# ELEKTRONN/ELEKTRONN2

Measured on AMD Instinct MI355X. Metric: training_input_voxels_per_sec, higher is better.
Workload: dtype f32; 1 GPU; neuro3d_lite (1,1,23,183,183)->(1,2,10,37,37) fwd+bwd+Adam, 1 sample/GPU; parallelism=dp1, hipgraph=True, steps_per_launch=10

## Files before the change

elektronn2_amd/backend.py:

```python
from __future__ import annotations

import ctypes as C
import os
from typing import Optional, Sequence

import numpy as np
import torch

_HERE = os.path.dirname(os.path.abspath(__file__))
LIB_PATH = os.environ.get("E2HIP_LIB") or os.path.join(_HERE, "libe2hip.so")

ACT = {"lin": 0, "linear": 0, "relu": 1, "tanh": 2, "sigmoid": 3, "sig": 3, "logistic": 3,
       "abs": 4, "elu": 5, "selu": 6, "soft+": 7}


class E2Error(RuntimeError):
    pass


POOL_MODE = {'avg': 1, 'sum': 2}


class Tensor5(C.Structure):
    _fields_ = [("ptr", C.c_void_p),
# ... 69 lines not shown
        "e2_conv3d_wgrad_acc": (C.c_int, [vp, P5, P5, fp, i, i, i]),
        "e2_conv3d_wgrad_pad": (C.c_int, [vp, P5, P5, fp, i, i, i, i]),
        "e2_pack_job_bytes": (sz, []),
        "e2_pack_job_fill": (C.c_int, [vp, fp, vp, i, i, i, i, i, i]),
        "e2_pack_job_set_rows": (C.c_int, [vp, i]),
        "e2_pack_job_set_stride": (C.c_int, [vp, i]),
        "e2_set_image_rows": (C.c_int, [vp, i]),
        "e2_conv3d_pack_multi": (C.c_int, [vp, vp, i]),
        "e2_conv3d_pack_multi_ex": (C.c_int, [vp, vp, i, i]),
        "e2_head_supported": (C.c_int, [i, i]),
        "e2_head_fwd": (C.c_int, [vp, P5, fp, fp, i, P5, P5, fp]),
        "e2_head_bwd_workspace_bytes": (C.c_size_t, [i, i, i, i, i, i]),
        "e2_tail_supported": (C.c_int, [i, i, i]),
        "e2_tail_workspace_bytes": (C.c_size_t, [i, i, i, i, i, i, i]),
        "e2_tail_fwd_bwd": (C.c_int, [vp, P5, fp, fp, fp, i, fp, fp, i, P5, P5, P5, P5, i, P5, fp, fp,
                                      C.c_void_p, C.c_size_t, C.POINTER(C.c_int)]),
        "e2_tail_reduce": (C.c_int, [vp, C.c_void_p, i, i, i, fp, fp, fp, fp, fp, i, fp]),
        "e2_head_bwd": (C.c_int, [vp, P5, fp, P5, P5, fp, P5, i, fp, fp, fp, C.c_void_p,
                                  C.c_size_t]),
        "e2_malis_loss_weights": (C.c_int, [i, C.c_void_p, i, C.c_void_p, C.c_void_p,
                                            C.c_void_p, i, C.c_void_p]),
        "e2_malis_connected_components": (C.c_int, [i, i, C.c_void_p, C.c_void_p, C.c_void_p,
                                                    i, C.c_void_p]),
        "e2_warp_slice": (C.c_int, [vp, P5, C.POINTER(C.c_float), i, C.c_uint,
                                    C.POINTER(C.c_int), C.POINTER(C.c_float), P5]),
        "e2_grey_augment": (C.c_int, [vp, fp, C.c_size_t, C.c_float, C.c_float, C.c_float]),
        "e2_stream_fork": (C.c_int, [vp, C.c_void_p]),
        "e2_stream_join": (C.c_int, [vp, C.c_void_p]),
        "e2_conv1_supported": (C.c_int, [i, i, i, i, i, i, i]),
        "e2_conv1_pool_act_fwd": (C.c_int, [vp, P5, fp, fp, i, i, i, i, i, i, P5]),
        "e2_conv1_bwd_workspace_bytes": (C.c_size_t, [i, i, i, i, i, i, i]),
        "e2_conv1_pool_act_bwd": (C.c_int, [vp, P5, fp, fp, P5, i, i, i, i, i, fp, fp,
                                            C.c_void_p, C.c_size_t]),
        "e2_pool_bias_act_fwd": (C.c_int, [vp, P5, fp, i, i, i, i, P5]),
        "e2_conv3d_fwd_packed_parts": (C.c_int, [vp, P5, vp, i, i, i, i, P5, C.c_int64, i,
                                                 C.POINTER(C.c_int)]),
        "e2_conv3d_dgrad_packed_parts": (C.c_int, [vp, P5, vp, i, i, i, i, P5, C.c_int64, i,
                                                   C.POINTER(C.c_int)]),
        "e2_pool_bias_act_fwd_parts": (C.c_int, [vp, P5, C.c_int64, i, fp, i, i, i, i, P5]),
        "e2_pool_bias_act_bwd_parts": (C.c_int, [vp, P5, C.c_int64, i, P5, fp, i, i, i, i, P5, fp]),
        "e2_bias_act_bwd_out_parts": (C.c_int, [vp, P5, C.c_int64, i, P5, i, P5, fp]),
        "e2_pool_bias_act_bwd": (C.c_int, [vp, P5, P5, fp, i, i, i, i, P5, fp]),
        "e2_maxpool3d_fwd": (C.c_int, [vp, P5, i, i, i, P5]),
        "e2_maxpool3d_bwd": (C.c_int, [vp, P5, P5, i, i, i, P5, i]),
        "e2_pool3d_lin_fwd": (C.c_int, [vp, P5, i, i, i, i, i, i, i, P5]),
        "e2_pool3d_lin_bwd": (C.c_int, [vp, P5, i, i, i, i, i, i, i, P5, i]),
        "e2_upconv3d_workspace_bytes": (sz, [i, i, i, i, i, i, i, i, i]),
        "e2_upconv3d_fwd": (C.c_int, [vp, P5, fp, fp, i, i, i, i, i, P5, vp, sz]),
        "e2_upconv3d_bwd": (C.c_int, [vp, P5, fp, P5, P5, i, i, i, i, P5, fp, fp, vp, sz]),
        "e2_upconv3d_image_bytes": (sz, [i, i, i, i, i]),
        "e2_upconv3d_fwd_packed": (C.c_int, [vp, P5, fp, fp, i, i, i, i, i, P5]),
        "e2_upconv3d_bwd_packed": (C.c_int, [vp, P5, fp, P5, P5, i, i, i, i, P5, fp, fp, vp, sz, i]),
        "e2_transpose_ncdhw_to_ndhwc": (C.c_int, [vp, P5, fp]),
        "e2_transpose_ndhwc_to_ncdhw": (C.c_int, [vp, fp, P5]),
        "e2_copy5": (C.c_int, [vp, P5, P5, i]),
        "e2_set_dgrad_zinset": (C.c_int, [vp, i]),
        "e2_pad5": (C.c_int, [vp, P5, P5, i, i, i, C.c_float, i]),
        "e2_fill": (C.c_int, [vp, fp, sz, C.c_float]),
        "e2_softmax_nll_fwd": (C.c_int, [vp, P5, P5, P5, fp]),
        "e2_softmax_nll_bwd": (C.c_int, [vp, P5, P5, fp, P5, fp]),
        "e2_softmax_nll_fwd_w": (C.c_int, [vp, P5, P5, P5, fp, PW]),
        "e2_softmax_nll_bwd_w": (C.c_int, [vp, P5, P5, fp, P5, fp, PW]),
        "e2_softmax_nll_grouped_fwd": (C.c_int, [vp, P5, P5, P5, i, fp]),
        "e2_softmax_nll_grouped_bwd": (C.c_int, [vp, P5, P5, i, fp, P5, fp]),
        "e2_head_fwd_w": (C.c_int, [vp, P5, fp, fp, i, P5, P5, fp, PW]),
        "e2_head_bwd_w": (C.c_int, [vp, P5, fp, P5, P5, fp, P5, i, fp, fp, fp, C.c_void_p,
# ... 380 lines not shown
                                          int(getattr(jobs_dev, 'max_taps', 248))),
             "e2_conv3d_pack_multi_ex")

    @staticmethod
    def conv1_supported(cin, k, pool):
        return bool(_lib.e2_conv1_supported(cin, k[0], k[1], k[2], pool[0], pool[1], pool[2]))

    def conv1_pool_act_fwd(self, x, w, bias, pool, act, out):
        _chk(_lib.e2_conv1_pool_act_fwd(self.h, C.byref(t5(x)), _fp(w), _fp(bias), w.shape[0],
                                        w.shape[3], w.shape[4], pool[1], pool[2], ACT[act],
                                        C.byref(t5(out))), "e2_conv1_pool_act_fwd")

    def conv1_pool_act_fwd_bf16(self, x, w, bias, pool, act, out, next_xb, next_kg):
        _chk(_lib.e2_conv1_pool_act_fwd_bf16(self.h, C.byref(t5(x)), _fp(w), _fp(bias), w.shape[0],
                                             w.shape[3], w.shape[4], pool[1], pool[2], ACT[act],
                                             C.byref(t5(out)), C.c_void_p(next_xb.data_ptr()),
                                             int(next_kg)), "e2_conv1_pool_act_fwd_bf16")

    @staticmethod
    def conv1_bwd_ws_bytes(dout_shape, k):
        n, cout, d, ho, wo = (int(v) for v in dout_shape)
        return int(_lib.e2_conv1_bwd_workspace_bytes(n, cout, d, ho, wo, k[1], k[2]))

    def conv1_pool_act_bwd(self, x, w, bias, dout, pool, act, dw, dbias, ws=None):
        if ws is None:
            ws = torch.empty(self.conv1_bwd_ws_bytes(dout.shape, w.shape[2:]) // 4 + 16,
                             dtype=torch.float32, device=self.device)
        _chk(_lib.e2_conv1_pool_act_bwd(self.h, C.byref(t5(x)), _fp(w), _fp(bias),
                                        C.byref(t5(dout)), w.shape[3], w.shape[4], pool[1],
                                        pool[2], ACT[act], _fp(dw), _fp(dbias),
                                        C.c_void_p(ws.data_ptr()), ws.numel() * 4),
             "e2_conv1_pool_act_bwd")

    def pool_bias_act_fwd(self, y, bias, pool, act, out):
        _chk(_lib.e2_pool_bias_act_fwd(self.h, C.byref(t5(y)), _fp(bias), pool[0], pool[1],
                                       pool[2], ACT[act], C.byref(t5(out))),
             "e2_pool_bias_act_fwd")

    def pool_bias_act_bwd(self, dout, y, bias, pool, act, dy, dbias):
        _chk(_lib.e2_pool_bias_act_bwd(self.h, C.byref(t5(dout)), C.byref(t5(y)), _fp(bias),
                                       pool[0], pool[1], pool[2], ACT[act], C.byref(t5(dy)),
                                       _fp(dbias)), "e2_pool_bias_act_bwd")

    def act_fwd(self, pre, bias, act, out):
        _chk(_lib.e2_act_fwd(self.h, C.byref(t5(pre)), _fp(bias), ACT[act], C.byref(t5(out))),
             "e2_act_fwd")

    def loss_partials(self, pred):
        n = int(_lib.e2_loss_partials(self.h, C.byref(t5(pred))))
        if n <= 0:
            raise E2Error("e2_loss_partials: empty prediction %s" % (tuple(pred.shape),))
        return n

    def loss_fwd(self, term, pred, sig, target, partials):
        if partials.numel() < 4 * self.loss_partials(pred):
            raise E2Error("loss_fwd: the partials slab is too small for this prediction")
        _chk(_lib.e2_loss_fwd(self.h, C.byref(term), C.byref(t5(pred)),
                              None if sig is None else C.byref(t5(sig)), C.byref(t5(target)),
                              _fp(partials)), "e2_loss_fwd")

    def loss_mix(self, terms, partials, n_tot, mix, coef, term_loss, count, loss_out):
        k = len(terms)
        if not (len(partials) == len(n_tot) == k):
            raise E2Error("loss_mix: %d terms, %d slabs, %d sizes" % (k, len(partials), len(n_tot)))
        if k > MAX_LOSS_TERMS:
            raise E2Error("loss_mix: %d terms, at most %d are supported" % (k, MAX_LOSS_TERMS))
# ... 473 lines not shown
```

elektronn2_amd/csrc/conv_first.hip:

```cpp
#include "common.hpp"
#include <algorithm>

struct First {
  const float* x;
  const float* w;
  const float* bias;
  float* out;
  const float* dout;
  float* dw;
  float* dbias;
  int N, Cout, D, Ho, Wo;
  long xsN, xsD, xsH;
  long osN, osC, osD, osH;
  int act;
  int tilesX, tilesY;
};

template <int KH, int KW, int PY, int PX>
__device__ __forceinline__ float first_conv(const float (&win)[PY + KH - 1][PX + KW - 1],
                                            const float* __restrict__ wc, int a, int b) {
  float s = 0.f;
#pragma unroll
  for (int ty = 0; ty < KH; ++ty)
#pragma unroll
// ... 220 lines not shown

static int conv1_fwd(e2_ctx* ctx, const e2_tensor5* x, const float* w, const float* bias, int cout,
                     int kh, int kw, int py, int px, int act, const e2_tensor5* out, void* next_xb,
                     int next_kg) {
  E2_REQUIRE(ctx && w && bias, "conv1_pool_act_fwd: null argument");
  const int v = first_supported(1, kh, kw, 1, py, px);
  E2_REQUIRE(v, "conv1_pool_act_fwd: unsupported kernel/pool %dx%d / %dx%d", kh, kw, py, px);
  First p{};
  if (int rc = first_fill(p, x, out, cout, kh, kw, py, px, "conv1_pool_act_fwd")) return rc;
  p.w = w; p.bias = bias; p.out = out->ptr; p.act = act;
  if (e2i_firstm_mg(cout) && (next_xb || !e2_dbg_env("E2_FIRST_VALU")))
    return e2i_firstm_fwd(ctx, v, x, w, bias, cout, py, px, act, out, next_xb, next_kg);
  E2_REQUIRE(!next_xb, "conv1_pool_act_fwd_bf16: %d output channels (matrix-core form: <= 32)", cout);
  const long nTiles = (long)p.N * p.D * p.tilesY * p.tilesX;
  const int grid = (int)std::min<long>(nTiles, ctx->num_cu * 8);
  if (v == 1)
    hipLaunchKernelGGL((first_fwd_kernel<4, 4, 2, 2>), dim3(grid), dim3(256), 0, ctx->stream, p, (int)nTiles);
  else if (v == 2)
    hipLaunchKernelGGL((first_fwd_kernel<6, 6, 2, 2>), dim3(grid), dim3(256), 0, ctx->stream, p, (int)nTiles);
  else
    hipLaunchKernelGGL((first_fwd_kernel<3, 3, 1, 1>), dim3(grid), dim3(256), 0, ctx->stream, p, (int)nTiles);
  E2_CHECK_HIP(hipGetLastError());
  return 0;
}

extern "C" size_t e2_conv1_bwd_workspace_bytes(int n, int cout, int d, int ho, int wo, int kh,
                                               int kw) {
  const long tiles = (long)n * d * e2_cdiv(ho, 8) * e2_cdiv(wo, 32);
  const long tilesM = (long)n * d * e2_cdiv(ho, 4) * e2_cdiv(wo * 2, 64);
  const size_t valu = (size_t)tiles * cout * (kh * kw + 1);
  return sizeof(float) * std::max(valu, e2i_firstm_ws_floats(tilesM, cout, kh * kw));
}

extern "C" int e2_conv1_pool_act_bwd(e2_ctx* ctx, const e2_tensor5* x, const float* w,
                                     const float* bias, const e2_tensor5* dout, int kh, int kw,
                                     int py, int px, int act, float* dw, float* dbias,
                                     void* ws, size_t ws_bytes) {
  E2_REQUIRE(ctx && w && bias && dw && dbias && ws, "conv1_pool_act_bwd: null argument");
  const int v = first_supported(1, kh, kw, 1, py, px);
  E2_REQUIRE(v, "conv1_pool_act_bwd: unsupported kernel/pool %dx%d / %dx%d", kh, kw, py, px);
  First p{};
  if (int rc = first_fill(p, x, dout, dout ? dout->c : 0, kh, kw, py, px, "conv1_pool_act_bwd"))
    return rc;
  p.w = w; p.bias = bias; p.dout = dout->ptr; p.dw = dw; p.dbias = dbias; p.act = act;
  const long nTiles = (long)p.N * p.D * p.tilesY * p.tilesX;
  E2_REQUIRE(nTiles < (1L << 31), "conv1_pool_act_bwd: too many tiles");
  E2_REQUIRE(ws_bytes >= e2_conv1_bwd_workspace_bytes(p.N, p.Cout, p.D, p.Ho, p.Wo, kh, kw),
             "conv1_pool_act_bwd: workspace too small");
  float* part = (float*)ws;
  if (e2i_firstm_mg(p.Cout) && !e2_dbg_env("E2_FIRST_VALU")) {
    int nslots = 0;
    if (int rc = e2i_firstm_bwd(ctx, v, x, w, bias, dout, py, px, act, part, &nslots)) return rc;
    const int T = kh * kw, total = p.Cout * (T + 1);
    hipLaunchKernelGGL(first_bwd_reduce_sm_kernel, dim3(e2_cdiv(total, 4)), dim3(256), 0, ctx->stream,
                       part, nslots, p.Cout, T, dw, dbias);
    E2_CHECK_HIP(hipGetLastError());
    return 0;
  }
  if (v == 1)
    hipLaunchKernelGGL((first_bwd_kernel<4, 4, 2, 2>), dim3((int)nTiles), dim3(256), 0, ctx->stream, p, part);
  else if (v == 2)
    hipLaunchKernelGGL((first_bwd_kernel<6, 6, 2, 2>), dim3((int)nTiles), dim3(256), 0, ctx->stream, p, part);
  else
    hipLaunchKernelGGL((first_bwd_kernel<3, 3, 1, 1>), dim3((int)nTiles), dim3(256), 0, ctx->stream, p, part);
  E2_CHECK_HIP(hipGetLastError());
  const int T = kh * kw, total = p.Cout * (T + 1);
  const int slices = (int)std::min<long>(nTiles, 64);
  hipLaunchKernelGGL(first_bwd_reduce_kernel, dim3(e2_cdiv(total, 256), slices), dim3(256), 0,
                     ctx->stream, part, (int)nTiles, p.Cout, T, dw, dbias);
  E2_CHECK_HIP(hipGetLastError());
  return 0;
}
```

elektronn2_amd/csrc/tail.hip:

```cpp
#include "common.hpp"
#include "nll_w.hpp"
#include <algorithm>
#include <vector>

typedef float f32x4 __attribute__((ext_vector_type(4)));
typedef __attribute__((address_space(3))) void* lds_vp;
typedef const __attribute__((address_space(1))) void* gbl_vp;

namespace {

constexpr int kMT = 13;
constexpr int kRows = 16 * kMT;

struct TailP {
  const float* x; long xsN, xsC;
  const float* wpf; int coPf, ciPf;
  const float* wpd; int coPd, ciPd;
  const float* b1;
  const float* wh; const float* bh;
  const float* tg; long tsN;
  float* pr; long psN, psC;
  float* dpre; long dsN, dsC;
  float* dx; long gsN, gsC, gsD, gsH;
  int H, W;
// ... 88 lines not shown
    const float tv = tp[i];
#pragma unroll
    for (int c = 0; c < NC; ++c) cnt += (tv == (float)c) ? Lc[c] : 0.f;
  }
#pragma unroll
  for (int o = 32; o > 0; o >>= 1) cnt += __shfl_xor(cnt, o, 64);
  if (blockIdx.x == 0 && blockIdx.y == 0 && threadIdx.x == 0) cnt += head_w_count_dn(wt, N * NC, S);
  if ((threadIdx.x & 63) == 0 && cnt != 0.f) unsafeAtomicAdd(stats + 1, cnt);
}

__global__ __launch_bounds__(256) void tail_reduce_kernel(const float* __restrict__ part, int nWG,
                                                          int nc, int c2, float* dwh, float* dbh,
                                                          float* db1, float* stats, float* loss_out,
                                                          float* count_out, int c1gm, float* dbp) {
  const int psz = tail_psz(nc, c2, c1gm);
  const int idx = blockIdx.x * 4 + (threadIdx.x >> 6), lane = threadIdx.x & 63;
  if (idx >= psz) return;
  const float* row = part + (long)idx * nWG;
  float s = 0.f;
  for (int b = lane; b < nWG; b += 64) s += row[b];
#pragma unroll
  for (int o = 32; o > 0; o >>= 1) s += __shfl_xor(s, o, 64);
  if (lane != 0) return;
  if (idx == nc * c2 + nc + c2) {
    stats[0] = s;
    if (loss_out) loss_out[0] = s / (stats[1] + E2_EPS_NLL);
    if (count_out) count_out[0] = stats[1];
    return;
  }
  float* dst = idx < nc * c2 ? dwh + idx
             : (idx < nc * c2 + nc ? dbh + (idx - nc * c2)
             : (idx < nc * c2 + nc + c2 ? db1 + (idx - nc * c2 - nc) : dbp + (idx - nc * c2 - nc - c2 - 1)));
  *dst += s;
}

bool flat_sp(const e2_tensor5* t) {
  return t->sh == t->w && t->sd == (int64_t)t->h * t->w;
}
bool same_sp(const e2_tensor5* a, const e2_tensor5* b) {
  return a->n == b->n && a->d == b->d && a->h == b->h && a->w == b->w;
}

void tail_cfg(const e2_ctx* ctx, long N, long S, int* wm, int* kc) {
  const long cus = ctx ? ctx->num_cu : 256;
  if (N * ((S + 31) / 32) >= cus) { *wm = 2; *kc = 16; }
  else if (N * ((S + 31) / 32) >= cus / 2) { *wm = 2; *kc = 40; }
  else { *wm = 4; *kc = 40; }
#ifdef E2_DEBUG_ENV
  if (const char* f = e2_dbg_env("E2_TAIL_CFG")) sscanf(f, "%d,%d", wm, kc);
#endif
}
long tail_grid(long N, long S, int wm) {
  const int np = 16 * (4 / wm);
  return N * ((S + np - 1) / np);
}

template <int WM, int NC, int KC>
int launch_tail_w(e2_ctx* ctx, const TailP& p, const NllW& wt, long grid) {
  constexpr size_t ldsb = tail_lds_bytes<WM, NC, KC>();
  static bool attr_done = false;
  if (!attr_done) {
    E2_CHECK_HIP(hipFuncSetAttribute(reinterpret_cast<const void*>(&tail_w_kernel<WM, NC, KC>),
                                     hipFuncAttributeMaxDynamicSharedMemorySize, 160 * 1024));
    attr_done = true;
  }
  hipLaunchKernelGGL((tail_w_kernel<WM, NC, KC>), dim3((unsigned)grid), dim3(256), ldsb, ctx->stream, p, wt);
// ... 155 lines not shown
                               const float* w_head, const float* b_head, int ncls,
                               const e2_tensor5* target, const e2_tensor5* probs,
                               const e2_tensor5* dpre, const e2_tensor5* dx, int gm_mode,
                               const e2_tensor5* gm_src, const float* gm_bias, float* stats,
                               void* ws, size_t ws_bytes, int* n_slots) {
  return tail_fwd_bwd_impl(ctx, x, wp_fwd, wp_dgrad, bias1, c2, w_head, b_head, ncls, target, probs,
                           dpre, dx, gm_mode, gm_src, gm_bias, stats, ws, ws_bytes, n_slots, nullptr);
}

extern "C" int e2_tail_fwd_bwd_w(e2_ctx* ctx, const e2_tensor5* x, const float* wp_fwd,
                                 const float* wp_dgrad, const float* bias1, int c2,
                                 const float* w_head, const float* b_head, int ncls,
                                 const e2_tensor5* target, const e2_tensor5* probs,
                                 const e2_tensor5* dpre, const e2_tensor5* dx, int gm_mode,
                                 const e2_tensor5* gm_src, const float* gm_bias, float* stats,
                                 void* ws, size_t ws_bytes, int* n_slots,
                                 const e2_nll_weights* wts) {
  return tail_fwd_bwd_impl(ctx, x, wp_fwd, wp_dgrad, bias1, c2, w_head, b_head, ncls, target, probs,
                           dpre, dx, gm_mode, gm_src, gm_bias, stats, ws, ws_bytes, n_slots, wts);
}

extern "C" int e2_tail_reduce(e2_ctx* ctx, const void* ws, int n_slots, int c2, int ncls,
                              float* dw_head, float* db_head, float* db1, float* stats,
                              float* loss_out, int c1_gm, float* db_parent) {
  E2_REQUIRE(ctx && ws && dw_head && db_head && db1 && stats && n_slots > 0, "tail_reduce: bad argument");
  E2_REQUIRE(c1_gm >= 0 && (c1_gm == 0 || db_parent), "tail_reduce: the parent's bias gradient is missing");
  const int psz = tail_psz(ncls, c2, c1_gm);
  hipLaunchKernelGGL(tail_reduce_kernel, dim3(e2_cdiv(psz, 4)), dim3(256), 0,
                     ctx->stream, (const float*)ws, n_slots, ncls, c2, dw_head, db_head, db1, stats,
                     loss_out, ctx->loss_count_out, c1_gm, db_parent);
  E2_CHECK_HIP(hipGetLastError());
  return 0;
}
```

elektronn2_amd/neuromancer/loss.py:

```python
from __future__ import annotations

import numpy as np

from .graphutils import TaggedShape, floatX
from .node_basic import Node, Sym
from .variables import VariableParam

__all__ = ['Softmax', 'MultinoulliNLL', 'MalisNLL', 'SquaredLoss', 'AbsLoss', 'BinaryNLL',
           'GaussianNLL', 'AggregateLoss', 'Classification', 'Errors']

MAX_LOSS_TERMS = 8

EPS = 1e-5


class Softmax(Node):
    def __init__(self, parent, n_class='auto', n_indep=1, name="softmax", print_repr=True):
        super(Softmax, self).__init__(parent, name, print_repr)
        n_f = parent.shape['f']
        if hasattr(parent, 'activation_func'):
            if parent.activation_func != 'lin':
                raise ValueError("The parent of a Softmax-node must have a "
                                 "linear activation function.")
        if n_class == 'auto':
# ... 186 lines not shown
                kw = dict(gm_mode=gm[0], gm_src=gm[1], gm_bias=gm[2])
            with plan.loss_grad_mode():
                plan.scratch[self, 'tail_slots'] = plan.ctx.tail_fwd_bwd(
                    plan.out[par], plan.scratch[tail, 'wp_f'], plan.scratch.get((tail, 'wp_d')),
                    plan.param(tail.b), plan.param(head.w).reshape(head.n_f, -1),
                    plan.param(head.b), plan.out[self.target], plan.out[self.pred],
                    plan.scratch[tail, 'dy'], dx, stats, plan.scratch[tail, 'tail_ws'],
                    weights=self._weights(plan), **kw)
            return
        plan.zero_early(stats)
        head = self.pred._head(plan)
        if head is not None:
            plan.ctx.head_fwd(plan.out[head.parent], plan.param(head.w), plan.param(head.b),
                              plan.out[self.target], plan.out[self.pred], stats,
                              weights=self._weights(plan))
            return
        if self.n_indep != 1:
            plan.ctx.softmax_nll_grouped_fwd(plan.out[self.pred.parent], plan.out[self.target],
                                             plan.out[self.pred], self.n_indep, stats)
            return
        plan.ctx.softmax_nll_fwd(plan.out[self.pred.parent], plan.out[self.target],
                                 plan.out[self.pred], stats, weights=self._weights(plan))

    def _plan_bwd(self, plan):
        with plan.loss_grad_mode():
            self._plan_bwd_launches(plan)

    def _plan_bwd_launches(self, plan):
        head = self.pred._head(plan)
        tail = self._tail(plan)
        if tail is not None:
            par = tail.parent
            gm = tail._tail_gm(plan) if plan.needs_grad(par) else None
            plan.ctx.tail_reduce(plan.scratch[tail, 'tail_ws'], plan.scratch[self, 'tail_slots'],
                                 tail.n_f, head.n_f, plan.pgrad(head.w).reshape(head.n_f, -1),
                                 plan.pgrad(head.b), plan.pgrad(tail.b),
                                 plan.scratch[self.pred, 'stats'], plan.scratch[self, 'loss'],
                                 db_parent=plan.pgrad(par.b) if gm is not None else None)
            return
        if head is not None:
            dst, first = (plan.grad_slot(head.parent) if plan.needs_grad(head.parent)
                          else (None, True))
            plan.ctx.head_bwd(plan.out[head.parent], plan.param(head.w), plan.out[self.pred],
                              plan.out[self.target], plan.scratch[self.pred, 'stats'], dst,
                              not first, plan.pgrad(head.w), plan.pgrad(head.b),
                              plan.scratch[self, 'loss'], ws=plan.scratch[self, 'head_ws'],
                              weights=self._weights(plan))
            return
        logits = self.pred.parent
        dst, first = plan.grad_slot(logits)
        if not first:
            raise NotImplementedError("logits consumed by several nodes")
        if self.n_indep != 1:
            plan.ctx.softmax_nll_grouped_bwd(plan.out[self.pred], plan.out[self.target],
                                             self.n_indep, plan.scratch[self.pred, 'stats'], dst,
                                             plan.scratch[self, 'loss'])
            return
        plan.ctx.softmax_nll_bwd(plan.out[self.pred], plan.out[self.target],
                                 plan.scratch[self.pred, 'stats'], dst,
                                 plan.scratch[self, 'loss'], weights=self._weights(plan))

    def loss_value(self, plan):
        s = plan.scratch[self.pred, 'stats']
        return s[0] / (s[1] + EPS)


class MalisNLL(Node):

    def __init__(self, pred, aff_gt, seg_gt, nhood, unrestrict_neg=True, class_weights=None,
                 example_weights=None, name="nll", print_repr=True):
        super(MalisNLL, self).__init__([pred, aff_gt, seg_gt], name, print_repr)
# ... 380 lines not shown
```

elektronn2_amd/neuromancer/neural.py:

```python
from __future__ import annotations

import logging

import numpy as np

from .graphutils import floatX, TaggedShape
from .. import autotune
from . import bf16_ahead
from .node_basic import Node, Concat, Add, Sym
from .variables import VariableWeight, ConstantParam, VariableParam

logger = logging.getLogger('elektronn2log')

__all__ = ['Conv', 'UpConv', 'Pool', 'Crop', 'Pad', 'AutoMerge', 'UpConvMerge', 'NeuralLayer',
           'FragmentsToDense', 'Perceptron']

_PLAIN_ACTS = ('relu', 'lin', 'linear')
_HIP_ACTS = _PLAIN_ACTS + ('tanh', 'sigmoid', 'sig', 'logistic', 'abs', 'elu', 'selu', 'soft+')


def check_activation(activation_func):
    if activation_func not in _HIP_ACTS:
        raise NotImplementedError("activation_func=%r: only %s are on the HIP hot path"
                                  % (activation_func, _HIP_ACTS))
# ... 651 lines not shown
                ctx.act_fwd(out, None, self.activation_func, out)
            return
        if not self._plain_act():
            out = plan.out[self]
            if all(p == 1 for p in self._p3):
                ctx.act_fwd(y, plan.param(self.b), self.activation_func, out)
            elif (self, 'lin') in plan.scratch:
                ctx.maxpool3d_fwd(y, self._p3, plan.scratch[self, 'lin'])
                ctx.act_fwd(plan.scratch[self, 'lin'], plan.param(self.b), self.activation_func, out)
            else:
                ctx.pool_bias_act_fwd(y, plan.param(self.b), self._p3, 'lin', out)
                ctx.act_fwd(out, None, self.activation_func, out)
            return
        ndst = bf16_ahead.next_dst(plan, self)
        if ndst is not None:
            ctx.pool_bias_act_fwd_bf16(yp[0], plan.param(self.b), self._p3, self.activation_func,
                                       plan.out[self], ndst, parts=y_nparts, part_stride=yp.stride(0))
            plan._xb_ready[plan.bf16a[self, 'next']['consumer']] = True
        elif y_nparts > 1:
            ctx.pool_bias_act_fwd_parts(yp, y_nparts, plan.param(self.b), self._p3,
                                        self.activation_func, plan.out[self])
        else:
            ctx.pool_bias_act_fwd(y, plan.param(self.b), self._p3, self.activation_func,
                                  plan.out[self])

    def _plan_bwd(self, plan):
        ctx = plan.ctx
        if self._fused_head(plan) is not None:
            return
        x = self._x(plan)
        if self._fused_first(plan):
            if plan.opt['side_join_first']:
                plan.join_side()
            ctx.conv1_pool_act_bwd(x, self._w5(plan.param(self.w)), plan.param(self.b), plan.grad[self],
                                   self._p3, self.activation_func, plan.pgrad(self.w),
                                   plan.pgrad(self.b), ws=plan.scratch[self, 'ws1'])
            return
        dy = plan.scratch[self, 'dy']
        tail = self._tail(plan) is not None
        if tail:
            if plan.needs_grad(self.parent):
                plan.grad_slot(self.parent)
                if self._tail_gm(plan) is not None:
                    plan.scratch[self.parent, 'dy_by_tail'] = True
        elif self._bn():
            train = self.batch_normalisation == 'train'
            pooled = any(p != 1 for p in self._p3)
            lin = plan.scratch[self, 'lin'] if pooled else plan.scratch[self, 'y']
            dlin = plan.scratch[self, 'dlin'] if pooled else dy
            if not self._plain_act():
                ctx.act_bwd(plan.grad[self], plan.scratch[self, 'pre'], None, self.activation_func,
                            plan.grad[self], None)
            ctx.batchnorm_act_bwd(plan.grad[self], lin, plan.param(self.gamma),
                                  plan.param(self.b), plan.scratch[self, 'bn_save'], train,
                                  self._lin_act(), dlin,
                                  plan.pgrad(self.gamma) if self.gamma.apply_train else None,
                                  plan.pgrad(self.b))
            if pooled:
                ctx.maxpool3d_bwd(dlin, plan.scratch[self, 'y'], self._p3, dy)
        elif not self._plain_act():
            g = plan.grad[self]
            if all(p == 1 for p in self._p3):
                ctx.act_bwd(g, plan.scratch[self, 'y'], plan.param(self.b), self.activation_func,
                            dy, plan.pgrad(self.b))
            else:
                dlin = plan.scratch[self, 'dlin']
                ctx.act_bwd(g, plan.scratch[self, 'lin'], plan.param(self.b),
                            self.activation_func, dlin, plan.pgrad(self.b))
                ctx.maxpool3d_bwd(dlin, plan.scratch[self, 'y'], self._p3, dy)
# ... 633 lines not shown
```

elektronn2_amd/neuromancer/options.py:

```python
import contextlib
import os


def _b(v):
    return str(v).strip().lower() not in ("0", "", "false", "off", "no")


def _tri(v):
    return None if v is None or str(v) == "" else _b(v)


SPEC = {
    "graph": ("E2_NO_GRAPH", lambda v: not _b(v), True,
              "capture the step into hipGraphs after one eager call (E2_NO_GRAPH=1 turns it off)"),
    "side_stream": ("E2_SIDE_STREAM", _tri, None,
                    "weight gradients on a second stream; None = only in bf16 mode (DESIGN finding 7)"),
    "side_join_first": ("E2_SIDE_JOIN_FIRST", _b, False,
                        "side stream on: the fused first layer's backward waits for the weight gradients on the "
                        "side stream (it runs 62 instead of 35 us beside them, VERDICT r4 weak 9) -- measured: "
                        "bf16 lite183 0.813 -> 0.821 ms, neuro3d 1.144 -> 1.149, unet132 equal: the overlap is "
                        "worth more than the slowdown; off"),
    "side_defer": ("E2_SIDE_DEFER", _b, True,
                   "side stream on: a weight gradient's launches are ISSUED behind the main stream's next "
                   "launches (same dependencies): in the captured graph the main chain then stays on one "
# ... 16 lines not shown
    "fuse_tail": ("E2_FUSE_TAIL", _b, True, "last 1x1x1 conv + head + loss in one launch (finding 33)"),
    "bf16_tail": ("E2_BF16_TAIL", _b, True,
                  "bf16 mode: the tail launch too (its two GEMMs round their operands in registers)"),
    "tail_gm": ("E2_TAIL_GM", _b, True, "the tail launch carries its parent's activation backward"),
    "upconv_packed": ("E2_UPCONV_PACKED", _b, True, "UpConv weight images packed by the plan's one repack launch"),
    "concat_alias": ("E2_CONCAT_ALIAS", _b, True, "a concat hands channel slices to parents only it consumes"),
    "pad_inplace": ("E2_PAD_INPLACE", _b, True,
                    "a 'same' / 'full' conv finds its parent's output inside its zero-framed input image "
                    "wherever the parent's producing launch writes a strided view (no pad launch); off: "
                    "every such conv pads by one e2_pad5 launch per step"),
    "zero_in_update": ("E2_ZERO_IN_UPDATE", _b, True, "the optimiser launch clears the gradient arena (finding 38)"),
    "image_stride": ("E2_IMAGE_STRIDE", _b, True,
                     "once a conv launch's tiling is known its packed weight image gets rows as long as that "
                     "tiling's tiles reach (+ 16), not the any-tiling formula (e2_set_image_rows; finding 52)"),
    "pack_rows": ("E2_PACK_ROWS", _b, False,
                  "the repack rewrites the padding rows the TUNED tiling of each launch fetches, not the "
                  "worst case over all tilings (e2_pack_job_set_rows): the repack itself 31 -> 24 us on "
                  "neuro3d, in the step -7 us (neuro3d), -13 us (unet3d_lite), +6 us (neuro3d_lite), "
                  "+-0 (unet3d) -- below the gate; off (DESIGN finding 51)"),
    "adam_pack": ("E2_ADAM_PACK", _b, False,
                  "the Adam launch writes the packed weight images (e2_adam_pack_step); measured slower "
                  "than the two launches it replaces (DESIGN finding 46): off"),
    "dp_overlap": ("E2_DP_OVERLAP", _b, True, "exchange the late layers' gradients under the early backward"),
    "dp_fused_scale": ("E2_DP_FUSED_SCALE", _b, True, "collectives only sum, the optimiser kernel normalises"),
    "bf16_ahead": ("E2_BF16_AHEAD", _b, True, "bf16 mode: producers write the GEMM operands (finding 43)"),
    "bf16_ahead_min": ("E2_BF16_AHEAD_MIN", float, 0.0,
                       "... only when this share of the GEMM launches are memory forms (round 4: 0.6, neuro3d's "
                       "11 of 25 stayed out; with the side stream on a queue of its own -- finding 54 -- engaging "
                       "them pays there too: neuro3d 0.948 -> 0.930 ms, unet3d 6.12 -> 5.84, neuro3d_lite 0.682 -> "
                       "0.640; unet3d_lite 2.44 -> 2.47 is the one that loses)"),
    "bf16_ahead_wgrad_only": ("E2_BF16_AHEAD_WGRAD_ONLY", _b, False, "... gradient images for the weight gradient alone"),
    "bf16_xkeep": ("E2_BF16_XKEEP", _b, True, "bf16 mode: the forward's channels-last copy of x serves the wgrad"),
    "bf16_wpack": ("E2_BF16_WPACK", str, "step", "'step': one filter-row pack launch per step; 'call': per launch"),
    "dense_act_gib": ("E2_DENSE_ACT_GIB", float, 48.0, "activation budget of tiled dense prediction (GiB)"),
}

_set = {}


def get(name):
    if name in _set:
        return _set[name]
    env, parse, default, _ = SPEC[name]
    v = os.environ.get(env)
    return default if v is None else parse(v)


def snapshot(overrides=None):
    d = {k: get(k) for k in SPEC}
    for k, v in (overrides or {}).items():
        if k not in SPEC:
            raise KeyError("unknown plan option %r (known: %s)" % (k, ", ".join(sorted(SPEC))))
        d[k] = v
    return d


def set_plan_options(**kw):
    reset = kw.pop("reset", ())
    for k in reset:
        _set.pop(k, None)
    for k, v in kw.items():
        if k not in SPEC:
            raise KeyError("unknown plan option %r (known: %s)" % (k, ", ".join(sorted(SPEC))))
        if v is None and k != "side_stream":
            _set.pop(k, None)
        else:
# ... 13 lines not shown
```

elektronn2_amd/neuromancer/plan.py:

```python
from __future__ import annotations

import os

import numpy as np
import torch

from .. import backend

_ctx = None


def get_ctx():
    global _ctx
    if _ctx is None:
        import os
        from .. import parallel
        dev = parallel.local_device()
        _ctx = backend.Context(dev)
        if os.environ.get("E2_MFMA_DTYPE", "f32") not in ("f32", "float32"):
            _ctx.set_mfma_dtype(os.environ["E2_MFMA_DTYPE"])
    return _ctx


def set_mfma_dtype(dtype):
# ... 380 lines not shown
        order = dict((id(n), i) for i, n in enumerate(self.model.dropout_nodes()))
        self._drop_ordinal = dict((n, order[id(n)]) for n in self._drop_nodes)
        if self._drop_nodes:
            self.model.dropout_state_dev()
        with torch.cuda.stream(self.stream):
            offs, tot = [], 0
            for n in self.inputs:
                offs.append(tot)
                tot += (int(np.prod(self.out_shape(n))) + 3) // 4 * 4
            self.input_arena = self.empty_flat(max(tot, 4))
            self.input_slices = {}
            for n, o in zip(self.inputs, offs):
                sh = self.out_shape(n)
                self.out[n] = self.input_arena[o:o + int(np.prod(sh))].view(sh)
                self.input_slices[n] = (o, int(np.prod(sh)))
            for n in self.nodes:
                n._plan_alloc(self)
            if getattr(self.ctx, 'mfma_dtype', 'f32') == 'bf16':
                self._bf16_ws_alloc()
            self._pack_dev = self._pack_dev_up = self._upd = None
            if self.pack_jobs:
                jobs = [(self._w5(self.param(w)), wp, mode) for (w, wp, mode) in self.pack_jobs]
                self._pack_dev = self.ctx.make_pack_jobs(jobs)
                self._plan_fused_update(jobs)
        self._graphs = None
        self._segs = None
        self._segs_key = None
        self._dp_scale_mode = False
        self._seg_idx = 0
        self._zero_seen, self._zero_batched, self._zero_keep = [], {}, None
        self._capturing = False
        self._calls = 0
        self._grad_written = set()
        self._ev_pairs = [(self.ctx.event(), self.ctx.event()), (self.ctx.event(), self.ctx.event())]
        self._ev_idx = 0
        self._n_runs = 0
        self._async = None
        self._ring = None
        self._hist = None
        self._step_state = None
        self._multi = {}
        self._built = True

    @property
    def _ev0(self):
        return self._ev_pairs[self._ev_idx][0]

    @property
    def _ev1(self):
        return self._ev_pairs[self._ev_idx][1]

    def _plan_fused_update(self, jobs):
        if self.step != 'Adam' or not self.opt['adam_pack']:
            return
        m = self.model
        by_param, order, up = {}, [], []
        for (w, wp, mode), (w5, _, _) in zip(self.pack_jobs, jobs):
            if mode in (0, 1):
                if id(w) not in by_param:
                    if not getattr(w, 'apply_train', False) or id(w) not in m._slots:
                        return
                    by_param[id(w)] = [w, tuple(int(v) for v in w5.shape), None, None]
                    order.append(id(w))
                by_param[id(w)][2 + mode] = wp
            else:
                up.append((w5, wp, mode))
# ... 91 lines not shown
            def packs():
                self.ctx.conv3d_pack_multi(*self._pack_dev)
                if self.use_side and self.opt['wb_on_side']:
                    self.ensure_wb()
            self.on_side(packs, always=True)
        drop = self._drop_ids
        for n in self.nodes:
            n._plan_fwd(self)
            if id(n) in drop:
                n._drop_fwd(self)
        self.join_side()

    def ensure_wb(self):
        if not self._wb_ready and self._bf16_wjobs is not None and \
                self.opt['bf16_wpack'] == "step":
            self.ctx.conv3d_bf16_pack_w_multi(*self._bf16_wjobs)
            self._wb_ready = True
        return self._wb_ready

    def _bwd_nodes(self):
        return [n for n in reversed(self.nodes)
                if id(n) in self._loss_anc and (self.needs_grad(n) or n is self.loss_node)]

    def _emit_backward(self, part=None):
        nodes = self._bwd_nodes()
        if part is not None:
            k = self._dp_cut()[0]
            nodes = nodes[:k] if part == 0 else nodes[k:]
        if part in (None, 0):
            if not self._upd_zeroes_g():
                self.zero_early(self.model.G)
            self._grad_written = set()
        drop = self._drop_ids
        for n in nodes:
            if id(n) in drop:
                n._drop_bwd(self)
            n._plan_bwd(self)
        self.join_side()

    def _dp_cut(self):
        if self._dp_cut_cache is not False:
            return self._dp_cut_cache
        self._dp_cut_cache = None
        m = self.model
        if not self.opt['dp_overlap'] or m.n_train < (1 << 16):
            return None
        nodes = self._bwd_nodes()
        last = {}
        for i, n in enumerate(nodes):
            for p in n.params.values():
                if getattr(p, 'apply_train', False) and id(p) in m._slots:
                    last[id(p)] = i
        slots = sorted(((m._slots[q][0], q) for q in last), reverse=True)
        for k in range(1, len(nodes) - 1):
            lo = m.n_train
            for off, q in slots:
                if last[q] >= k:
                    break
                lo = off
            if m.n_train - lo >= 0.75 * m.n_train:
                self._dp_cut_cache = (k, lo)
                break
        return self._dp_cut_cache

    def _labelled_count(self):
        ln = self.loss_node
        kids = ln.parent if isinstance(ln.parent, (list, tuple)) else [ln.parent]
        if len(kids) != 1 or type(kids[0]).__name__ != 'MultinoulliNLL':
            return None
        st = self.scratch.get((kids[0].pred, 'stats'))
        return None if st is None else st[1:2]
# ... 425 lines not shown
```

include/e2hip.h:

```cpp
#ifndef E2HIP_H
#define E2HIP_H

#include <stddef.h>
#include <stdint.h>

#ifdef __cplusplus
extern "C" {
#endif

typedef struct e2_ctx e2_ctx;

typedef struct e2_tensor5 {
  float*  ptr;
  int32_t n, c, d, h, w;
  int64_t sn, sc, sd, sh;
} e2_tensor5;

enum { E2_ACT_LIN = 0, E2_ACT_RELU = 1, E2_ACT_TANH, E2_ACT_SIGMOID, E2_ACT_ABS,
       E2_ACT_ELU, E2_ACT_SELU, E2_ACT_SOFTPLUS };
enum { E2_MFMA_F32 = 0, E2_MFMA_BF16 = 1 };
enum { E2_TILING_IGEMM = 0, E2_TILING_WGRAD = 1 };

int  e2_ctx_create(int device, e2_ctx** out);
int  e2_ctx_destroy(e2_ctx* ctx);
// ... 28 lines not shown
int e2_bias_act_bwd_out(e2_ctx*, const e2_tensor5* dout, const e2_tensor5* out, int act,
                        const e2_tensor5* dy, float* dbias);
int e2_conv3d_dgrad_packed_actbwd(e2_ctx*, const e2_tensor5* dy_pad, const void* wp, int cin,
                                  int kd, int kh, int kw, const e2_tensor5* out_prev,
                                  int act_prev, const float* bias_prev,
                                  const e2_tensor5* dy_pad_prev, int pd, int ph, int pw,
                                  float* dbias_prev);

int e2_conv3d_wgrad(e2_ctx*, const e2_tensor5* x, const e2_tensor5* dy,
                    float* dw, int kd, int kh, int kw);
int e2_conv3d_wgrad_acc(e2_ctx*, const e2_tensor5* x, const e2_tensor5* dy,
                        float* dw, int kd, int kh, int kw);
int e2_conv3d_wgrad_pad(e2_ctx*, const e2_tensor5* x, const e2_tensor5* dy_pad,
                        float* dw, int kd, int kh, int kw, int accumulate);

size_t e2_pack_job_bytes(void);
int e2_pack_job_fill(void* rec, const float* w, void* wp, int cout, int cin,
                     int kd, int kh, int kw, int mode);
int e2_set_image_rows(e2_ctx* ctx, int rows);
int e2_pack_job_set_stride(void* rec, int rows);
int e2_pack_job_set_rows(void* rec, int rows);
int e2_conv3d_pack_multi(e2_ctx*, const void* jobs_dev, int njobs);
int e2_conv3d_pack_multi_ex(e2_ctx*, const void* jobs_dev, int njobs, int max_taps);

int e2_conv1_supported(int cin, int kd, int kh, int kw, int pz, int py, int px);
int e2_conv1_pool_act_fwd(e2_ctx*, const e2_tensor5* x, const float* w,
                          const float* bias, int cout, int kh, int kw, int py,
                          int px, int act, const e2_tensor5* out);
size_t e2_conv1_bwd_workspace_bytes(int n, int cout, int d, int ho, int wo, int kh, int kw);
int e2_conv1_pool_act_bwd(e2_ctx*, const e2_tensor5* x, const float* w,
                          const float* bias, const e2_tensor5* dout, int kh,
                          int kw, int py, int px, int act, float* dw, float* dbias,
                          void* ws, size_t ws_bytes);

int e2_conv3d_fwd_packed_parts(e2_ctx*, const e2_tensor5* x, const void* wp, int cout, int kd,
                               int kh, int kw, const e2_tensor5* y, int64_t part_stride,
                               int max_parts, int* nparts);
int e2_conv3d_dgrad_packed_parts(e2_ctx*, const e2_tensor5* dy_pad, const void* wp, int cin,
                                 int kd, int kh, int kw, const e2_tensor5* dx,
                                 int64_t part_stride, int max_parts, int* nparts);
int e2_pool_bias_act_fwd_parts(e2_ctx*, const e2_tensor5* y, int64_t part_stride, int nparts,
                               const float* bias, int pz, int py, int px, int act,
                               const e2_tensor5* out);
int e2_pool_bias_act_bwd_parts(e2_ctx*, const e2_tensor5* dout, int64_t dout_part_stride,
                               int dout_parts, const e2_tensor5* y, const float* bias, int pz,
                               int py, int px, int act, const e2_tensor5* dy, float* dbias);
int e2_bias_act_bwd_out_parts(e2_ctx*, const e2_tensor5* dout, int64_t dout_part_stride,
                              int dout_parts, const e2_tensor5* out, int act,
                              const e2_tensor5* dy, float* dbias);

int e2_pool_bias_act_fwd(e2_ctx*, const e2_tensor5* y, const float* bias,
                         int pz, int py, int px, int act,
                         const e2_tensor5* out);
int e2_pool_bias_act_bwd(e2_ctx*, const e2_tensor5* dout, const e2_tensor5* y,
                         const float* bias, int pz, int py, int px, int act,
                         const e2_tensor5* dy, float* dbias);

int e2_maxpool3d_fwd(e2_ctx*, const e2_tensor5* x, int pz, int py, int px,
                     const e2_tensor5* out);
int e2_maxpool3d_bwd(e2_ctx*, const e2_tensor5* dout, const e2_tensor5* x,
                     int pz, int py, int px, const e2_tensor5* dx,
                     int accumulate);

enum { E2_POOL_AVG = 1, E2_POOL_SUM = 2 };
int e2_pool3d_lin_fwd(e2_ctx*, const e2_tensor5* x, int pz, int py, int px, int sz, int sy,
                      int sx, int mode, const e2_tensor5* out);
// ... 28 lines not shown
int e2_pad5(e2_ctx*, const e2_tensor5* src, const e2_tensor5* dst, int pz, int py, int px,
            float value, int frame_only);

int e2_fill_multi(e2_ctx*, const void* ptrs_dev, const void* counts_dev, int nregions,
                  float value);
int e2_set_skip_zero_fill(e2_ctx*, int on);

int e2_step_prologue(e2_ctx*, const float* ring, int n_slots, size_t slot_floats, float* dst,
                     const float* src, int n_vals, float* hist, int hist_slots, void* state);
int e2_set_input_slack(e2_ctx*, int bytes);
int e2_conv_last_zero_fill(const e2_ctx*, void** ptr, size_t* n);
int e2_set_dgrad_zinset(e2_ctx*, int planes);

int e2_head_supported(int cin, int ncls);
int e2_head_fwd(e2_ctx*, const e2_tensor5* x, const float* w, const float* bias, int ncls,
                const e2_tensor5* target, const e2_tensor5* probs, float* stats);
size_t e2_head_bwd_workspace_bytes(int n, int cin, int ncls, int d, int h, int w);
int e2_head_bwd(e2_ctx*, const e2_tensor5* x, const float* w, const e2_tensor5* probs,
                const e2_tensor5* target, const float* stats, const e2_tensor5* dx,
                int accumulate_dx, float* dw, float* dbias, float* loss_out, void* ws,
                size_t ws_bytes);

int e2_tail_supported(int c1, int c2, int ncls);
size_t e2_tail_workspace_bytes(int n, int c1, int c2, int ncls, int d, int h, int w);
int e2_tail_fwd_bwd(e2_ctx*, const e2_tensor5* x, const float* wp_fwd, const float* wp_dgrad,
                    const float* bias1, int c2, const float* w_head, const float* b_head,
                    int ncls, const e2_tensor5* target, const e2_tensor5* probs,
                    const e2_tensor5* dpre, const e2_tensor5* dx, int gm_mode,
                    const e2_tensor5* gm_src, const float* gm_bias, float* stats, void* ws,
                    size_t ws_bytes, int* n_slots);
int e2_tail_reduce(e2_ctx*, const void* ws, int n_slots, int c2, int ncls, float* dw_head,
                   float* db_head, float* db1, float* stats, float* loss_out, int c1_gm,
                   float* db_parent);

int e2_softmax_nll_fwd(e2_ctx*, const e2_tensor5* logits,
                       const e2_tensor5* target, const e2_tensor5* probs,
                       float* stats);
int e2_softmax_nll_bwd(e2_ctx*, const e2_tensor5* probs,
                       const e2_tensor5* target, const float* stats,
                       const e2_tensor5* dlogits, float* loss_out);

int e2_softmax_nll_grouped_fwd(e2_ctx*, const e2_tensor5* logits, const e2_tensor5* target,
                               const e2_tensor5* probs, int n_indep, float* stats);
int e2_softmax_nll_grouped_bwd(e2_ctx*, const e2_tensor5* probs, const e2_tensor5* target,
                               int n_indep, const float* stats, const e2_tensor5* dlogits,
                               float* loss_out);

typedef struct e2_nll_weights {
  const float*      class_w;
  const e2_tensor5* example_w;
  const float*      labelled;
  const float*      not_present;
} e2_nll_weights;
int e2_softmax_nll_fwd_w(e2_ctx*, const e2_tensor5* logits, const e2_tensor5* target,
                         const e2_tensor5* probs, float* stats, const e2_nll_weights* wts);
int e2_softmax_nll_bwd_w(e2_ctx*, const e2_tensor5* probs, const e2_tensor5* target,
                         const float* stats, const e2_tensor5* dlogits, float* loss_out,
                         const e2_nll_weights* wts);
int e2_head_fwd_w(e2_ctx*, const e2_tensor5* x, const float* w, const float* bias, int ncls,
                  const e2_tensor5* target, const e2_tensor5* probs, float* stats,
                  const e2_nll_weights* wts);
int e2_head_bwd_w(e2_ctx*, const e2_tensor5* x, const float* w, const e2_tensor5* probs,
                  const e2_tensor5* target, const float* stats, const e2_tensor5* dx,
                  int accumulate_dx, float* dw, float* dbias, float* loss_out, void* ws,
                  size_t ws_bytes, const e2_nll_weights* wts);
int e2_tail_fwd_bwd_w(e2_ctx*, const e2_tensor5* x, const float* wp_fwd, const float* wp_dgrad,
// ... 163 lines not shown
```

Baseline: 520.8 million voxels/s.

## Defer tail slot reduction and fuse it with first-layer wgrad reduction launch

Adds a combined kernel that reduces both the tail's per-workgroup partial sums and the first conv layer's per-slot weight/bias partials in one launch. In one-GPU Adam/SGD steps, the tail reduction is deferred from the head of the backward (ahead of the weight-gradient fork) to the end, where it shares the first layer's reduce launch. The aim is to remove one kernel launch and take a small reduction off the backward's critical chain. The cost is extra plumbing through the plan, and the loss/stats values are now written later in the step.

```diff
diff --git a/elektronn2_amd/backend.py b/elektronn2_amd/backend.py
--- a/elektronn2_amd/backend.py
+++ b/elektronn2_amd/backend.py
@@ -125,6 +125,10 @@
         "e2_conv1_bwd_workspace_bytes": (C.c_size_t, [i, i, i, i, i, i, i]),
         "e2_conv1_pool_act_bwd": (C.c_int, [vp, P5, fp, fp, P5, i, i, i, i, i, fp, fp,
                                             C.c_void_p, C.c_size_t]),
+        "e2_conv1_pool_act_bwd_slots": (C.c_int, [vp, P5, fp, fp, P5, i, i, i, i, i, fp, fp,
+                                                  C.c_void_p, C.c_size_t, C.POINTER(C.c_int)]),
+        "e2_tail_first_reduce": (C.c_int, [vp, C.c_void_p, i, i, i, fp, fp, fp, fp, fp, i, fp,
+                                           C.c_void_p, i, i, i, fp, fp]),
         "e2_pool_bias_act_fwd": (C.c_int, [vp, P5, fp, i, i, i, i, P5]),
         "e2_conv3d_fwd_packed_parts": (C.c_int, [vp, P5, vp, i, i, i, i, P5, C.c_int64, i,
                                                  C.POINTER(C.c_int)]),
@@ -571,6 +575,26 @@
                                         C.c_void_p(ws.data_ptr()), ws.numel() * 4),
              "e2_conv1_pool_act_bwd")
 
+    def conv1_pool_act_bwd_slots(self, x, w, bias, dout, pool, act, dw, dbias, ws):
+        n = C.c_int(0)
+        _chk(_lib.e2_conv1_pool_act_bwd_slots(self.h, C.byref(t5(x)), _fp(w), _fp(bias),
+                                              C.byref(t5(dout)), w.shape[3], w.shape[4], pool[1],
+                                              pool[2], ACT[act], _fp(dw), _fp(dbias),
+                                              C.c_void_p(ws.data_ptr()), ws.numel() * 4, C.byref(n)),
+             "e2_conv1_pool_act_bwd_slots")
+        return n.value
+
+    def tail_first_reduce(self, ws, n_slots, c2, ncls, dw_head, db_head, db1, stats, loss_out,
+                          db_parent, ws_first, n_slots_first, dw_first, db_first):
+        cout = int(dw_first.shape[0])
+        _chk(_lib.e2_tail_first_reduce(self.h, C.c_void_p(ws.data_ptr()), int(n_slots), int(c2),
+                                       int(ncls), _fp(dw_head), _fp(db_head), _fp(db1), _fp(stats),
+                                       _fp(loss_out) if loss_out is not None else None,
+                                       0 if db_parent is None else int(db_parent.numel()),
+                                       _fp(db_parent), C.c_void_p(ws_first.data_ptr()),
+                                       int(n_slots_first), cout, int(dw_first.numel()) // cout,
+                                       _fp(dw_first), _fp(db_first)), "e2_tail_first_reduce")
+
     def pool_bias_act_fwd(self, y, bias, pool, act, out):
         _chk(_lib.e2_pool_bias_act_fwd(self.h, C.byref(t5(y)), _fp(bias), pool[0], pool[1],
                                        pool[2], ACT[act], C.byref(t5(out))),
diff --git a/elektronn2_amd/csrc/conv_first.hip b/elektronn2_amd/csrc/conv_first.hip
--- a/elektronn2_amd/csrc/conv_first.hip
+++ b/elektronn2_amd/csrc/conv_first.hip
@@ -276,10 +276,26 @@
   return sizeof(float) * std::max(valu, e2i_firstm_ws_floats(tilesM, cout, kh * kw));
 }
 
+static int conv1_bwd(e2_ctx* ctx, const e2_tensor5* x, const float* w, const float* bias,
+                     const e2_tensor5* dout, int kh, int kw, int py, int px, int act, float* dw,
+                     float* dbias, void* ws, size_t ws_bytes, int* n_slots);
 extern "C" int e2_conv1_pool_act_bwd(e2_ctx* ctx, const e2_tensor5* x, const float* w,
                                      const float* bias, const e2_tensor5* dout, int kh, int kw,
                                      int py, int px, int act, float* dw, float* dbias,
                                      void* ws, size_t ws_bytes) {
+  return conv1_bwd(ctx, x, w, bias, dout, kh, kw, py, px, act, dw, dbias, ws, ws_bytes, nullptr);
+}
+extern "C" int e2_conv1_pool_act_bwd_slots(e2_ctx* ctx, const e2_tensor5* x, const float* w,
+                                           const float* bias, const e2_tensor5* dout, int kh,
+                                           int kw, int py, int px, int act, float* dw,
+                                           float* dbias, void* ws, size_t ws_bytes, int* n_slots) {
+  E2_REQUIRE(n_slots, "conv1_pool_act_bwd_slots: null n_slots");
+  *n_slots = 0;
+  return conv1_bwd(ctx, x, w, bias, dout, kh, kw, py, px, act, dw, dbias, ws, ws_bytes, n_slots);
+}
+static int conv1_bwd(e2_ctx* ctx, const e2_tensor5* x, const float* w, const float* bias,
+                     const e2_tensor5* dout, int kh, int kw, int py, int px, int act, float* dw,
+                     float* dbias, void* ws, size_t ws_bytes, int* n_slots) {
   E2_REQUIRE(ctx && w && bias && dw && dbias && ws, "conv1_pool_act_bwd: null argument");
   const int v = first_supported(1, kh, kw, 1, py, px);
   E2_REQUIRE(v, "conv1_pool_act_bwd: unsupported kernel/pool %dx%d / %dx%d", kh, kw, py, px);
@@ -295,6 +311,7 @@
   if (e2i_firstm_mg(p.Cout) && !e2_dbg_env("E2_FIRST_VALU")) {
     int nslots = 0;
     if (int rc = e2i_firstm_bwd(ctx, v, x, w, bias, dout, py, px, act, part, &nslots)) return rc;
+    if (n_slots) { *n_slots = nslots; return 0; }
     const int T = kh * kw, total = p.Cout * (T + 1);
     hipLaunchKernelGGL(first_bwd_reduce_sm_kernel, dim3(e2_cdiv(total, 4)), dim3(256), 0, ctx->stream,
                        part, nslots, p.Cout, T, dw, dbias);
diff --git a/elektronn2_amd/csrc/tail.hip b/elektronn2_amd/csrc/tail.hip
--- a/elektronn2_amd/csrc/tail.hip
+++ b/elektronn2_amd/csrc/tail.hip
@@ -144,6 +144,50 @@
              : (idx < nc * c2 + nc ? dbh + (idx - nc * c2)
              : (idx < nc * c2 + nc + c2 ? db1 + (idx - nc * c2 - nc) : dbp + (idx - nc * c2 - nc - c2 - 1)));
   *dst += s;
+}
+
+__global__ __launch_bounds__(256) void tail_first_reduce_kernel(const float* __restrict__ part, int nWG,
+                                                                int nc, int c2, float* dwh, float* dbh,
+                                                                float* db1, float* stats, float* loss_out,
+                                                                float* count_out, int c1gm, float* dbp,
+                                                                int nbT, const float* __restrict__ partF,
+                                                                int nSlotsF, int CoutF, int TF,
+                                                                float* dwF, float* dbF) {
+  const int lane = threadIdx.x & 63;
+  if ((int)blockIdx.x < nbT) {
+    const int psz = tail_psz(nc, c2, c1gm);
+    const int idx = blockIdx.x * 4 + (threadIdx.x >> 6);
+    if (idx >= psz) return;
+    const float* row = part + (long)idx * nWG;
+    float s = 0.f;
+    for (int b = lane; b < nWG; b += 64) s += row[b];
+#pragma unroll
+    for (int o = 32; o > 0; o >>= 1) s += __shfl_xor(s, o, 64);
+    if (lane != 0) return;
+    if (idx == nc * c2 + nc + c2) {
+      stats[0] = s;
+      if (loss_out) loss_out[0] = s / (stats[1] + E2_EPS_NLL);
+      if (count_out) count_out[0] = stats[1];
+      return;
+    }
+    float* dst = idx < nc * c2 ? dwh + idx
+               : (idx < nc * c2 + nc ? dbh + (idx - nc * c2)
+               : (idx < nc * c2 + nc + c2 ? db1 + (idx - nc * c2 - nc) : dbp + (idx - nc * c2 - nc - c2 - 1)));
+    *dst += s;
+    return;
+  }
+  const int idx = ((int)blockIdx.x - nbT) * 4 + (threadIdx.x >> 6);
+  if (idx >= CoutF * (TF + 1)) return;
+  const float* row = partF + (long)idx * nSlotsF;
+  float s = 0.f;
+#pragma unroll 4
+  for (int b = lane; b < nSlotsF; b += 64) s += row[b];
+#pragma unroll
+  for (int o = 32; o > 0; o >>= 1) s += __shfl_xor(s, o, 64);
+  if (lane != 0) return;
+  const int co = idx / (TF + 1), k = idx - co * (TF + 1);
+  if (k < TF) dwF[co * TF + (TF - 1 - k)] += s;
+  else dbF[co] += s;
 }
 
 bool flat_sp(const e2_tensor5* t) {
@@ -365,3 +409,22 @@
   E2_CHECK_HIP(hipGetLastError());
   return 0;
 }
+
+extern "C" int e2_tail_first_reduce(e2_ctx* ctx, const void* ws, int n_slots, int c2, int ncls,
+                                    float* dw_head, float* db_head, float* db1, float* stats,
+                                    float* loss_out, int c1_gm, float* db_parent,
+                                    const void* ws_first, int n_slots_first, int cout_first,
+                                    int taps_first, float* dw_first, float* db_first) {
+  E2_REQUIRE(ctx && ws && dw_head && db_head && db1 && stats && n_slots > 0, "tail_first_reduce: bad argument");
+  E2_REQUIRE(c1_gm >= 0 && (c1_gm == 0 || db_parent), "tail_first_reduce: the parent's bias gradient is missing");
+  E2_REQUIRE(ws_first && dw_first && db_first && n_slots_first > 0 && cout_first > 0 && taps_first > 0,
+             "tail_first_reduce: bad first-layer argument");
+  const int nbT = e2_cdiv(tail_psz(ncls, c2, c1_gm), 4);
+  const int nbF = e2_cdiv(cout_first * (taps_first + 1), 4);
+  hipLaunchKernelGGL(tail_first_reduce_kernel, dim3(nbT + nbF), dim3(256), 0, ctx->stream,
+                     (const float*)ws, n_slots, ncls, c2, dw_head, db_head, db1, stats, loss_out,
+                     ctx->loss_count_out, c1_gm, db_parent, nbT, (const float*)ws_first,
+                     n_slots_first, cout_first, taps_first, dw_first, db_first);
+  E2_CHECK_HIP(hipGetLastError());
+  return 0;
+}
diff --git a/elektronn2_amd/neuromancer/loss.py b/elektronn2_amd/neuromancer/loss.py
--- a/elektronn2_amd/neuromancer/loss.py
+++ b/elektronn2_amd/neuromancer/loss.py
@@ -242,11 +242,15 @@
         if tail is not None:
             par = tail.parent
             gm = tail._tail_gm(plan) if plan.needs_grad(par) else None
-            plan.ctx.tail_reduce(plan.scratch[tail, 'tail_ws'], plan.scratch[self, 'tail_slots'],
-                                 tail.n_f, head.n_f, plan.pgrad(head.w).reshape(head.n_f, -1),
-                                 plan.pgrad(head.b), plan.pgrad(tail.b),
-                                 plan.scratch[self.pred, 'stats'], plan.scratch[self, 'loss'],
-                                 db_parent=plan.pgrad(par.b) if gm is not None else None)
+            args = (plan.scratch[tail, 'tail_ws'], plan.scratch[self, 'tail_slots'],
+                    tail.n_f, head.n_f, plan.pgrad(head.w).reshape(head.n_f, -1),
+                    plan.pgrad(head.b), plan.pgrad(tail.b),
+                    plan.scratch[self.pred, 'stats'], plan.scratch[self, 'loss'],
+                    plan.pgrad(par.b) if gm is not None else None)
+            if plan.defer_tail_sums():
+                plan.tail_sums = args
+            else:
+                plan.ctx.tail_reduce(*args[:-1], db_parent=args[-1])
             return
         if head is not None:
             dst, first = (plan.grad_slot(head.parent) if plan.needs_grad(head.parent)
diff --git a/elektronn2_amd/neuromancer/neural.py b/elektronn2_amd/neuromancer/neural.py
--- a/elektronn2_amd/neuromancer/neural.py
+++ b/elektronn2_amd/neuromancer/neural.py
@@ -707,9 +707,14 @@
         if self._fused_first(plan):
             if plan.opt['side_join_first']:
                 plan.join_side()
-            ctx.conv1_pool_act_bwd(x, self._w5(plan.param(self.w)), plan.param(self.b), plan.grad[self],
-                                   self._p3, self.activation_func, plan.pgrad(self.w),
-                                   plan.pgrad(self.b), ws=plan.scratch[self, 'ws1'])
+            args = (x, self._w5(plan.param(self.w)), plan.param(self.b), plan.grad[self], self._p3,
+                    self.activation_func, plan.pgrad(self.w), plan.pgrad(self.b))
+            ws = plan.scratch[self, 'ws1']
+            if plan.tail_sums is not None:
+                n = ctx.conv1_pool_act_bwd_slots(*args, ws=ws)
+                plan.flush_tail_sums((ws, n, self._w5(plan.pgrad(self.w)), plan.pgrad(self.b)) if n else None)
+            else:
+                ctx.conv1_pool_act_bwd(*args, ws=ws)
             return
         dy = plan.scratch[self, 'dy']
         tail = self._tail(plan) is not None
diff --git a/elektronn2_amd/neuromancer/options.py b/elektronn2_amd/neuromancer/options.py
--- a/elektronn2_amd/neuromancer/options.py
+++ b/elektronn2_amd/neuromancer/options.py
@@ -72,6 +72,11 @@
     "bf16_ahead_wgrad_only": ("E2_BF16_AHEAD_WGRAD_ONLY", _b, False, "... gradient images for the weight gradient alone"),
     "bf16_xkeep": ("E2_BF16_XKEEP", _b, True, "bf16 mode: the forward's channels-last copy of x serves the wgrad"),
     "bf16_wpack": ("E2_BF16_WPACK", str, "step", "'step': one filter-row pack launch per step; 'call': per launch"),
+    "step_seams": ("E2_STEP_SEAMS", _b, True,
+                   "the one-GPU training step: the tail's slot sums leave the head of the backward -- the "
+                   "chain ahead of the weight gradients' fork -- and share the launch of the first layer's "
+                   "slot sums at its end (e2_tail_first_reduce; DESIGN finding 59).  The same sums bit for "
+                   "bit; off: e2_tail_reduce where it was, the first layer's backward with its own launch"),
     "dense_act_gib": ("E2_DENSE_ACT_GIB", float, 48.0, "activation budget of tiled dense prediction (GiB)"),
 }
 
diff --git a/elektronn2_amd/neuromancer/plan.py b/elektronn2_amd/neuromancer/plan.py
--- a/elektronn2_amd/neuromancer/plan.py
+++ b/elektronn2_amd/neuromancer/plan.py
@@ -436,6 +436,7 @@
         self._capturing = False
         self._calls = 0
         self._grad_written = set()
+        self._bwd_part, self.tail_sums = None, None
         self._ev_pairs = [(self.ctx.event(), self.ctx.event()), (self.ctx.event(), self.ctx.event())]
         self._ev_idx = 0
         self._n_runs = 0
@@ -593,11 +594,27 @@
                 self.zero_early(self.model.G)
             self._grad_written = set()
         drop = self._drop_ids
+        self._bwd_part, self.tail_sums = part, None
         for n in nodes:
             if id(n) in drop:
                 n._drop_bwd(self)
             n._plan_bwd(self)
+        self.flush_tail_sums()
         self.join_side()
+
+    def defer_tail_sums(self):
+        return (bool(self.opt['step_seams']) and self.step in ('Adam', 'SGD') and self._bwd_part is None
+                and self.model.dp_world() == 1)
+
+    def flush_tail_sums(self, first=None):
+        args, self.tail_sums = self.tail_sums, None
+        if args is None:
+            return False
+        if first is not None:
+            self.ctx.tail_first_reduce(*(args + first))
+        else:
+            self.ctx.tail_reduce(*args[:-1], db_parent=args[-1])
+        return True
 
     def _dp_cut(self):
         if self._dp_cut_cache is not False:
diff --git a/include/e2hip.h b/include/e2hip.h
--- a/include/e2hip.h
+++ b/include/e2hip.h
@@ -84,6 +84,10 @@
                           const float* bias, const e2_tensor5* dout, int kh,
                           int kw, int py, int px, int act, float* dw, float* dbias,
                           void* ws, size_t ws_bytes);
+int e2_conv1_pool_act_bwd_slots(e2_ctx*, const e2_tensor5* x, const float* w,
+                                const float* bias, const e2_tensor5* dout, int kh,
+                                int kw, int py, int px, int act, float* dw, float* dbias,
+                                void* ws, size_t ws_bytes, int* n_slots);
 
 int e2_conv3d_fwd_packed_parts(e2_ctx*, const e2_tensor5* x, const void* wp, int cout, int kd,
                                int kh, int kw, const e2_tensor5* y, int64_t part_stride,
@@ -178,6 +182,10 @@
 int e2_tail_reduce(e2_ctx*, const void* ws, int n_slots, int c2, int ncls, float* dw_head,
                    float* db_head, float* db1, float* stats, float* loss_out, int c1_gm,
                    float* db_parent);
+int e2_tail_first_reduce(e2_ctx*, const void* ws, int n_slots, int c2, int ncls, float* dw_head,
+                         float* db_head, float* db1, float* stats, float* loss_out, int c1_gm,
+                         float* db_parent, const void* ws_first, int n_slots_first,
+                         int cout_first, int taps_first, float* dw_first, float* db_first);
 
 int e2_softmax_nll_fwd(e2_ctx*, const e2_tensor5* logits,
                        const e2_tensor5* target, const e2_tensor5* probs,
```

Result: no change. 522.8 million voxels/s (median of 6 runs) (+0.4%).
